# lh3/minigraph

Measured on NVIDIA H100. Metric: mapped Gbp/s (-cx lr), higher is better.
Workload: dtype int64/u8 (fp32 chain penalties, bit-exact)

## Files before the change

### minigraph_b200/csrc/mgb_galign.cuh

```cuda
#pragma once
#include "mgb_pipeline.cuh"
#include "mgb_gchain.cuh"
#include "mgb_wfa_tiers.cuh"
#if defined(MGB_HOSTSIM)
#include <stdio.h>
#include <stdlib.h>
#endif

namespace mgb {

MG_HD inline int cigar_append1(Arena &A, AVec<uint64_t> &c, int32_t op, int32_t len)
{
	if (c.n > 0 && (int32_t)(c.a[c.n - 1] & 0xf) == op) c.a[c.n - 1] += (uint64_t)(int64_t)len << 4;
	else {
		uint64_t x = (uint64_t)(int64_t)len << 4 | (uint64_t)op;
		MGB_TRY(avec_push(A, c, x));
	}
	return 0;
}

MG_HD inline int cigar_append(Arena &A, AVec<uint64_t> &c, int32_t n_cigar, const uint32_t *cigar)
{
	if (n_cigar == 0) return 0;
	MGB_TRY(cigar_append1(A, c, (int32_t)(cigar[0] & 0xf), (int32_t)(cigar[0] >> 4)));
	MGB_TRY(avec_reserve(A, c, c.n + n_cigar - 1));
	for (int32_t k = 0; k < n_cigar - 1; ++k) c.a[c.n + k] = cigar[1 + k];
	c.n += n_cigar - 1;
	return 0;
}

struct CigarOut { uint64_t *cigar; int32_t n; };

struct WfaJob {
	int32_t rid, gc;
	int32_t l0, l;
	int32_t t_beg;
	int32_t t_last;
	int32_t tl, ql, q_off;
	int32_t n_cigar, status;
	int64_t lc_off;
	int64_t cig_off;
};

static const uint64_t PLAN_JOB = 1ULL << 63;
MG_HD inline unsigned long long *wfa_cig_chunk(int32_t *smem, int tier)
{
	static_assert(WfTier1::BYTES % 8 == 0 && WfTier1::BYTES + 16 <= WfTier1::STRIDE && WfTier2::BYTES % 8 == 0 && WfTier2::BYTES + 16 <= WfTier2::STRIDE, "no room for the slice state behind the tier layouts");
	return smem == 0 || tier > 2? (unsigned long long*)0 : (unsigned long long*)((char*)smem + (tier == 1? WfTier1::BYTES : WfTier2::BYTES));
}
static const unsigned long long CIG_CHUNK_BYTES = 2048;


MG_HD inline int wfa_job_run(Arena &A, const PipeCtx &c, int64_t job_idx, int lane, int32_t *smem, int tier, WfTbJob *tb)
{
	WfaJob *J = &c.jobs[job_idx];
	if (J->rid < 0) return 0;
	const int32_t rid = J->rid, l0 = J->l0, l = J->l, tl = J->tl, ql = J->ql;
	if (c.meta[rid].status < 0) return 0;
	const int32_t mlen = tl > ql? tl : ql;
	const int explore = (job_idx & 63) == 0;
	if (!explore && tier == 1 && mlen >= c.skip1_len) {
		if (lane == 0) {
			unsigned int at;
#if MGB_ON_DEVICE
			at = atomicAdd(&c.jobq_n[tier - 1], 1u);
#else
			at = c.jobq_n[tier - 1]++;
#endif
			c.jobq[tier - 1][at] = (int32_t)job_idx;
		}
		return 0;
	}
	const bool t2_long = tl > WfTier2::MAXLEN_ || ql > WfTier2::MAXLEN_;
	if ((tier == 1 && (tl > WfTier1::MAXLEN_ || ql > WfTier1::MAXLEN_)) || (tier == 2 && t2_long && !wf_ring_always_fits(tl, ql))) {
		if (lane == 0) {
			unsigned int at;
#if MGB_ON_DEVICE
			at = atomicAdd(&c.jobq_n[tier - 1], 1u);
#else
			at = c.jobq_n[tier - 1]++;
#endif
			c.jobq[tier - 1][at] = (int32_t)job_idx;
		}
		return 0;
	}
	const GraphDev &g = c.g;
	const LLChain *lc = (const LLChain*)(c.out + J->lc_off);
	const char *qs = c.b.seq + c.b.seq_off[rid] + J->q_off;
	const char *tseq;
	if (l == l0) tseq = g_vseq(g, lc[l0].v) + J->t_beg;
	else {
		char *seq;
		MGB_ALLOC(A, seq, char, tl + 1);
		int32_t n = g_vlen(g, lc[l0].v) - J->t_beg, at = 0;
		const char *s = g_vseq(g, lc[l0].v) + J->t_beg;
		for (int32_t x = lane; x < n; x += MGB_W) seq[at + x] = s[x];
		at += n;
		for (int32_t k = l0 + 1; k < l; ++k) {
			s = g_vseq(g, lc[k].v), n = g_vlen(g, lc[k].v);
			for (int32_t x = lane; x < n; x += MGB_W) seq[at + x] = s[x];
			at += n;
		}
		s = g_vseq(g, lc[l].v), n = J->t_last + 1;
		for (int32_t x = lane; x < n; x += MGB_W) seq[at + x] = s[x];
		at += n;
		if (at != tl) return MGB_E_INTERNAL;
		warp_sync();
		tseq = seq;
	}
	WfResult rst;
	unsigned long long pt0 = prof_clock();
	int rc;
	int64_t cont_cells = 0;
	if (tier == 1) rc = wfa_smem<WfTier1::W_, WfTier1::MAXLEN_, WfTier1::TBCAP_>(A, smem, tl, tseq, ql, qs, &rst, lane);
// ... 28 lines not shown
			c.jobq[tier - 1][at] = (int32_t)job_idx;
		}
		return 0;
	}
	if (rst.s < 0) return MGB_E_INTERNAL;
	wfa_tb_keep(tb, rst, tl, tseq, ql, qs, job_idx, lane);
	return 1;
}

MG_HD inline int wfa_job_finish(const PipeCtx &c, const WfTbJob &b, int32_t *smem, int tier, int lane)
{
	if (b.rc < 0) return b.rc;
	const int32_t n_cigar = b.n_cigar;
	const uint32_t *cigar = b.cig + b.first;
	int64_t coff = 0;
	if (lane == 0) {
#if MGB_ON_DEVICE
		unsigned long long *ck = wfa_cig_chunk(smem, tier);
		const unsigned long long need = ((unsigned long long)n_cigar * 4 + 15) & ~15ULL;
		if (ck == 0) coff = pool_alloc(c.pool_cig, (uint64_t)n_cigar * 4);
		else if (ck[0] + need > ck[1]) {
			const unsigned long long get = need > CIG_CHUNK_BYTES? need : CIG_CHUNK_BYTES;
			const int64_t off = pool_alloc(c.pool_cig, get);
			if (off < 0) ck[0] = ck[1] = 0;
			else ck[0] = (unsigned long long)off, ck[1] = (unsigned long long)off + get;
			coff = off;
		}
		if (ck && coff >= 0) coff = (int64_t)ck[0], ck[0] += need;
#else
		coff = pool_alloc(c.pool_cig, (uint64_t)n_cigar * 4);
#endif
	}
	coff = (int64_t)warp_bcast_u64((uint64_t)coff, 0);
	if (coff < 0) return MGB_E_POOL;
	uint32_t *dst = (uint32_t*)((char*)c.cig + coff);
	for (int32_t x = lane; x < n_cigar; x += MGB_W) dst[x] = cigar[x];
	if (lane == 0) { WfaJob *J = &c.jobs[b.job]; J->n_cigar = n_cigar, J->cig_off = coff; }
	return 0;
}

template<typename G>
struct WfaBatch {
	WfTbJob *rec;
	int32_t n;
	MG_HD void open(Arena &A)
	{
		A.top = 0, n = 0;
		rec = (WfTbJob*)arena_alloc(A, (uint64_t)MGB_W * sizeof(WfTbJob));
	}
	MG_HD void flush(const G &g, Arena &A, int lane)
	{
		if (n > 0) {
			const unsigned long long t0 = prof_clock();
			wfa_tb_batch(rec, n, lane);
			g.traced(prof_clock() - t0, lane);
			for (int32_t j = 0; j < n; ++j) {
				const WfTbJob &b = rec[j];
				const int rc = g.done(b, lane);
				if (rc < 0) g.fail(b.item, rc, lane);
			}
			warp_sync();
		}
		open(A);
	}
	MG_HD void add(const G &g, int item, Arena &A, int lane)
	{
		uint64_t mark = A.top;
		int rc = g.run(item, A, rec + n, lane);
		if (rc == MGB_E_ARENA && n > 0) {
			flush(g, A, lane);
			mark = A.top;
			rc = g.run(item, A, rec + n, lane);
		}
		if (rc < 0) g.fail(item, rc, lane);
		if (rc == 1) {
			if (lane == 0) rec[n].item = item;
			++n;
		} else A.top = mark;
		if (n == MGB_W || A.top > A.cap / 4) flush(g, A, lane);
	}
};


#if MGB_ON_DEVICE
MG_D inline void lane_atomic_add_u64(uint64_t *p, uint64_t v) { atomicAdd((unsigned long long*)p, (unsigned long long)v); }
#else
inline void lane_atomic_add_u64(uint64_t *p, uint64_t v) { *p += v; }
#endif

MG_HD inline int gchain_cigar_finish_w(Arena &A, const PipeCtx &c, GcSet &gt, CigarOut *out, int lane)
{
	const uint64_t FIRST = 1ULL << 62;
	for (int32_t i = 0; i < gt.n_gc; ++i) {
		GChain *gc = &gt.gc[i];
		const int32_t off_a0 = gt.lc[gc->off].off, n_plan = gc->n_plan;
		const uint64_t *plan = c.plan + gc->plan_off;
		int32_t *ioff;
		MGB_ALLOC(A, ioff, int32_t, n_plan + 1);
		int32_t tot = 0;
		for (int32_t base = 0; base < n_plan; base += MGB_W) {
			const int32_t t = base + lane;
			int32_t cnt = 0;
			if (t < n_plan) cnt = (plan[t] & PLAN_JOB)? c.jobs[plan[t] & ~PLAN_JOB].n_cigar : 1;
			const int32_t incl = warp_incl_scan_i32(cnt, lane);
			if (t < n_plan) ioff[t] = tot + incl - cnt;
			tot += warp_bcast_i32(incl, MGB_W - 1);
		}
		uint64_t *F, *O;
		int32_t *oidx;
		MGB_ALLOC(A, F, uint64_t, tot + 1);
		MGB_ALLOC(A, O, uint64_t, tot + 1);
		MGB_ALLOC(A, oidx, int32_t, tot + 1);
		warp_sync();
		for (int32_t t = lane; t < n_plan; t += MGB_W) {
			uint64_t *dst = F + ioff[t];
			if (plan[t] & PLAN_JOB) {
				const WfaJob *J = &c.jobs[plan[t] & ~PLAN_JOB];
				const uint32_t *cig = (const uint32_t*)((const char*)c.cig + J->cig_off);
				for (int32_t k = 0; k < J->n_cigar; ++k) dst[k] = (uint64_t)cig[k] | (k == 0? FIRST : 0);
			} else dst[0] = plan[t] | FIRST;
		}
		warp_sync();
		int32_t n_out = 0;
		for (int32_t base = 0; base < tot; base += MGB_W) {
			const int32_t j = base + lane;
			int head = 0;
			if (j < tot) head = j == 0 || !((F[j] & FIRST) && (F[j] & 0xf) == (F[j - 1] & 0xf));
			const uint32_t mh = warp_ballot(head);
			if (j < tot) {
				const int32_t o = n_out + mask_rank(mh, lane) + head - 1;
				oidx[j] = o;
				if (head) O[o] = F[j] & 0xf;
			}
			n_out += mask_count(mh);
		}
		warp_sync();
		for (int32_t j = lane; j < tot; j += MGB_W) lane_atomic_add_u64(&O[oidx[j]], (F[j] & ~FIRST) >> 4 << 4);
		warp_sync();
		int32_t mlen = 0, blen = 0, aplen = 0, l = 0;
		for (int32_t j = lane; j < n_out; j += MGB_W) {
			const int32_t op = (int32_t)(O[j] & 0xf), len = (int32_t)(O[j] >> 4);
			if (op == 7) mlen += len;
			blen += len;
			if (op != 1) aplen += len;
			if (op != 2) l += len;
		}
		mlen = warp_sum_i32(mlen), blen = warp_sum_i32(blen), aplen = warp_sum_i32(aplen), l = warp_sum_i32(l);
		if (lane == 0) {
			out[i].cigar = O, out[i].n = n_out;
			gc->has_cigar = 1;
			gc->n_cigar = n_out;
			gc->c_ss = (int32_t)gt.a[off_a0].x + 1 - (int32_t)(gt.a[off_a0].y >> 32 & 0xff);
			gc->c_ee = (int32_t)gt.a[off_a0 + gc->n_anchor - 1].x + 1;
			gc->c_mlen = mlen, gc->c_blen = blen, gc->c_aplen = aplen;
		}
		if (!(l == gc->qe - gc->qs && aplen == gc->pe - gc->ps)) return MGB_E_INTERNAL;
		warp_sync();
	}
	return 0;
}


struct DsOut { char *ds; int32_t len; int32_t *off; int32_t n_off; };

MG_HD inline char ds_nt(const char *s, int64_t i) { return "acgtn"[nt4((uint8_t)s[i])]; }

MG_HD inline char *ds_w_int(char *w, int32_t c)
{
	char buf[16];
	int l = 0;
	uint32_t x = c >= 0? (uint32_t)c : (uint32_t)(-c);
	do { buf[l++] = (char)(x % 10 + '0'); x /= 10; } while (x > 0);
	if (c < 0) buf[l++] = '-';
	for (int i = l - 1; i >= 0; --i) *w++ = buf[i];
	return w;
}

MG_HD inline char *ds_w_indel(char *w, int64_t len, const char *seq, int64_t ll, int64_t lr)
{
	int64_t i;
	if (ll + lr >= len) {
		*w++ = '[';
		for (i = 0; i < len; ++i) *w++ = ds_nt(seq, i);
		*w++ = ']';
	} else {
		int64_t k = 0;
		if (ll > 0) {
			*w++ = '[';
			for (i = 0; i < ll; ++i) *w++ = ds_nt(seq, k + i);
			*w++ = ']';
			k += ll;
		}
		for (i = 0; i < len - lr - ll; ++i) *w++ = ds_nt(seq, k + i);
		k += len - lr - ll;
		if (lr > 0) {
			*w++ = '[';
			for (i = 0; i < lr; ++i) *w++ = ds_nt(seq, k + i);
			*w++ = ']';
		}
	}
	return w;
}

static const int DS_CHUNKS = 32;
struct DsChunk { int64_t dx, dy; int32_t cap_b, cap_o, n_b, n_o; };

MG_HD inline int gchain_ds_w(Arena &A, const GraphDev &g, const char *qseq, GcSet &gt, const CigarOut *cg, DsOut *out, int lane)
{
	for (int32_t i = 0; i < gt.n_gc; ++i) {
		GChain *gc = &gt.gc[i];
		const uint64_t *cigar = cg[i].cigar;
		const int32_t n_cigar = gc->n_cigar, aplen = gc->c_aplen;
		char *seq;
		int64_t seq_l = 0;
		MGB_ALLOC(A, seq, char, aplen + 1);
		for (int32_t j = 0; j < gc->cnt; ++j) {
			const int32_t k = gc->off + j;
			const uint32_t v = gt.lc[k].v;
			const int32_t slen = g_vlen(g, v);
			const int32_t st = j > 0? 0 : gc->c_ss;
			const int32_t en = j < gc->cnt - 1? slen : gc->c_ee;
			if (seq_l + (en - st) > aplen) return MGB_E_INTERNAL;
			const char *s = g_vseq(g, v) + st;
			for (int32_t t = lane; t < en - st; t += MGB_W) seq[seq_l + t] = s[t];
			seq_l += en - st;
		}
		if (seq_l != aplen) return MGB_E_INTERNAL;
		DsChunk *ch;
		MGB_ALLOC(A, ch, DsChunk, DS_CHUNKS);
		const int32_t per = (n_cigar + DS_CHUNKS - 1) / DS_CHUNKS;
		for (int c = lane; c < DS_CHUNKS; c += MGB_W) {
			const int32_t j0 = c * per < n_cigar? c * per : n_cigar, j1 = j0 + per < n_cigar? j0 + per : n_cigar;
			DsChunk d;
			d.dx = d.dy = 0, d.cap_b = d.cap_o = d.n_b = d.n_o = 0;
			for (int32_t j = j0; j < j1; ++j) {
				const int64_t op = (int64_t)(cigar[j] & 0xf), len = (int64_t)(cigar[j] >> 4);
				if (op == 7) d.dx += len, d.dy += len, d.cap_b += 12, d.cap_o += 1;
				else if (op == 0 || op == 8) d.dx += len, d.dy += len, d.cap_b += (int32_t)(14 * len + 12), d.cap_o += (int32_t)(2 * len + 1);
				else if (op == 1) d.dy += len, d.cap_b += (int32_t)(len + 6), d.cap_o += 1;
				else if (op == 2) d.dx += len, d.cap_b += (int32_t)(len + 6), d.cap_o += 1;
			}
			ch[c] = d;
		}
		warp_sync();
		int64_t tot_cb = 0, tot_co = 0;
		for (int c = 0; c < DS_CHUNKS; ++c) tot_cb += ch[c].cap_b, tot_co += ch[c].cap_o;
		char *tmp_b;
		int32_t *tmp_o;
		MGB_ALLOC(A, tmp_b, char, tot_cb);
		MGB_ALLOC(A, tmp_o, int32_t, tot_co);
		int bad = 0;
		for (int c = lane; c < DS_CHUNKS; c += MGB_W) {
			const int32_t j0 = c * per < n_cigar? c * per : n_cigar, j1 = j0 + per < n_cigar? j0 + per : n_cigar;
			int64_t x = 0, y = gc->qs, cb = 0, co = 0;
			for (int q = 0; q < c; ++q) x += ch[q].dx, y += ch[q].dy, cb += ch[q].cap_b, co += ch[q].cap_o;
			char *const w0 = tmp_b + cb;
			char *w = w0;
			int32_t *const o0 = tmp_o + co;
			int32_t *o = o0;
			for (int32_t j = j0; j < j1; ++j) {
				const int64_t op = (int64_t)(cigar[j] & 0xf), len = (int64_t)(cigar[j] >> 4);
				if (op == 0 || op == 7 || op == 8) {
					int64_t z;
					int32_t l = 0;
					if (op == 7) l = (int32_t)len, z = len;
					else z = 0;
					for (; z < len; ++z) {
						const uint8_t cx = (uint8_t)nt4((uint8_t)seq[x + z]);
						const uint8_t cy = (uint8_t)nt4((uint8_t)qseq[y + z]);
						if (cx != cy) {
							if (l > 0) { *o++ = (int32_t)(w - w0); *w++ = ':'; w = ds_w_int(w, l); }
							*o++ = (int32_t)(w - w0);
							*w++ = '*', *w++ = "acgtn"[cx], *w++ = "acgtn"[cy];
							l = 0;
						} else ++l;
					}
					if (l > 0) { *o++ = (int32_t)(w - w0); *w++ = ':'; w = ds_w_int(w, l); }
					x += len, y += len;
				} else if (op == 1) {
					int64_t z, ll, lr;
					for (z = 1; z <= len; ++z)
						if (y - z < gc->qs || qseq[y + len - z] != qseq[y - z]) break;
					lr = z - 1;
					for (z = 0; z < len; ++z)
						if (y + len + z >= gc->qe || qseq[y + len + z] != qseq[y + z]) break;
					ll = z;
					*o++ = (int32_t)(w - w0);
					*w++ = '+';
					w = ds_w_indel(w, len, &qseq[y], ll, lr);
					y += len;
				} else if (op == 2) {
					int64_t z, ll, lr;
					for (z = 1; z <= len; ++z)
						if (x - z < 0 || seq[x + len - z] != seq[x - z]) break;
					lr = z - 1;
					for (z = 0; z < len; ++z)
						if (x + len + z >= aplen || seq[x + z] != seq[x + len + z]) break;
					ll = z;
					*o++ = (int32_t)(w - w0);
					*w++ = '-';
					w = ds_w_indel(w, len, &seq[x], ll, lr);
					x += len;
				}
			}
			ch[c].n_b = (int32_t)(w - w0), ch[c].n_o = (int32_t)(o - o0);
			if (ch[c].n_b > ch[c].cap_b || ch[c].n_o > ch[c].cap_o) bad = 1;
		}
		if (warp_any(bad)) return MGB_E_INTERNAL;
		warp_sync();
		int64_t tot_b = 0, tot_o = 0;
		for (int c = 0; c < DS_CHUNKS; ++c) tot_b += ch[c].n_b, tot_o += ch[c].n_o;
		char *str;
		int32_t *off;
		MGB_ALLOC(A, str, char, tot_b + 1);
		MGB_ALLOC(A, off, int32_t, tot_o);
		{
			int64_t cb = 0, co = 0, ab = 0, ao = 0;
			for (int c = 0; c < DS_CHUNKS; ++c) {
				const char *sb = tmp_b + cb;
				const int32_t *so = tmp_o + co;
				for (int32_t t = lane; t < ch[c].n_b; t += MGB_W) str[ab + t] = sb[t];
				for (int32_t t = lane; t < ch[c].n_o; t += MGB_W) off[ao + t] = so[t] + (int32_t)ab;
				cb += ch[c].cap_b, co += ch[c].cap_o, ab += ch[c].n_b, ao += ch[c].n_o;
			}
		}
		warp_sync();
		out[i].ds = str, out[i].len = (int32_t)tot_b, out[i].off = off, out[i].n_off = (int32_t)tot_o;
		if (lane == 0) gc->ds_len = (int32_t)tot_b, gc->n_dsoff = (int32_t)tot_o;
	}
	return 0;
}

struct ReadOut {
	int32_t status;
	int32_t n_gc, n_lc, n_a, rep_len;
	int32_t n_mz;
	uint32_t blob_size, blob2_size;
	int64_t blob_off;
	int64_t blob2_off;
};

MG_HD inline uint64_t align8(uint64_t x) { return (x + 7) & ~(uint64_t)7; }

struct GState {
	int32_t n_lc, n_u, n_gc, n_jobs;
	int64_t job_first;
};

MG_HD inline int stage_gchain_plan(const PipeCtx &c, ReadMeta &m, int rid, Arena &A, int32_t n_lc, LChain *lc, int32_t n_u, const uint64_t *u, const u128 *a, uint32_t *gc_hash)
{
	const MapOptDev &o = c.opt;
	int32_t n_gc = 0;
	int64_t job_first;
	{
		int64_t off = pool_alloc(c.pool_gjobs, (uint64_t)(n_lc > 0? n_lc : 1) * sizeof(GwfaJob));
		if (off < 0) return MGB_E_POOL;
		job_first = off / (int64_t)sizeof(GwfaJob);
	}
	struct LocalEmit {
		GwfaJob *dst; int rid; int32_t n, cap;
		MG_HD int operator()(GwfaJob &J) { if (n >= cap) return MGB_E_INTERNAL; J.rid = rid; dst[n++] = J; return 0; }
	} le;
	le.dst = c.gjobs + job_first, le.rid = rid, le.n = 0, le.cap = n_lc > 0? n_lc : 1;
	MGB_TRY(gchain_prep(c.g, n_u, u, lc, a, m.hash, o.min_gc_cnt, o.min_gc_score, o.gdp_max_ed, batch_n_seg(c.b, rid), gc_hash, &n_gc, le));
	for (int32_t i = le.n; i < le.cap; ++i) le.dst[i].rid = -1;
	uint64_t sz = sizeof(GState) + align8((uint64_t)n_lc * sizeof(LChain)) + (uint64_t)n_u * 8 + align8((uint64_t)n_gc * 4);
	int64_t goff = pool_alloc(c.pool_gstate, sz);
	if (goff < 0) return MGB_E_POOL;
	GState *gsb = (GState*)(c.gstate + goff);
	gsb->n_lc = n_lc, gsb->n_u = n_u, gsb->n_gc = n_gc, gsb->n_jobs = le.n, gsb->job_first = job_first;
	LChain *dlc = (LChain*)(gsb + 1);
	for (int32_t i = 0; i < n_lc; ++i) dlc[i] = lc[i];
	uint64_t *du = (uint64_t*)((char*)dlc + align8((uint64_t)n_lc * sizeof(LChain)));
	for (int32_t i = 0; i < n_u; ++i) du[i] = u[i];
	uint32_t *dh = (uint32_t*)(du + n_u);
	for (int32_t i = 0; i < n_gc; ++i) dh[i] = gc_hash[i];
	m.gstate_off = goff;
	return 0;
}

MG_HD inline int stage_gchain(const PipeCtx &c, ReadOut *routs, int rid, Arena &A, int lane)
{
	ReadMeta &m = c.meta[rid];
	ReadOut &ro = routs[rid];
	const MapOptDev &o = c.opt;
	if (lane == 0) ro.status = 0, ro.n_gc = ro.n_lc = ro.n_a = 0, ro.rep_len = m.rep_len, ro.n_mz = m.n_mz, ro.blob_size = ro.blob2_size = 0, ro.blob_off = ro.blob2_off = 0;
	if (m.status != 0) { if (lane == 0) ro.status = m.status; return 0; }
	const uint64_t mark = A.top;
	const int32_t qlen = c.b.seq_len[rid];
	const u128 *a = c.anchor + m.a_off;
	int32_t n_lc = m.n_lc, n_u = 0;
	uint64_t *u = 0;
	LChain *lc;
	uint32_t *gc_hash;
	MGB_ALLOC(A, lc, LChain, n_lc);
	MGB_ALLOC(A, gc_hash, uint32_t, n_lc);
	for (int32_t i = lane; i < n_lc; i += MGB_W) lc[i] = c.lchain[m.lc_off + i];
	warp_sync();
	unsigned long long pt0 = prof_clock();
	GcParam gp;
	gp.max_dist_g = gp.max_dist_q = gp.bw = o.bw_long, gp.ref_bonus = o.ref_bonus, gp.chn_pen_gap = o.chn_pen_gap, gp.mask_level = o.mask_level;
	MGB_TRY(gchain_dp_w(A, c.g, c.lab, &n_lc, lc, qlen, gp, o.max_gc_skip, a, &u, &n_u, lane));
	if (lane == 0) { unsigned long long dt = prof_clock() - pt0; prof_add(c, PROF_GC_DP_CYC, dt); prof_max(c, PROF_GC_DP_MAX_CYC, dt); }
	int rc = 0;
	if (lane == 0) {
		Arena B = A;
		rc = stage_gchain_plan(c, m, rid, B, n_lc, lc, n_u, u, a, gc_hash);
		if (B.peak > A.peak) A.peak = B.peak;
	}
	rc = warp_bcast_i32(rc, 0);
	A.top = mark;
	return rc;
}
// ... 136 lines not shown
	const MapOptDev &o = c.opt;
	if (m.status != 0) { ro.status = m.status; return 0; }
	uint64_t mark = A.top;
	const char *qseq = c.b.seq + c.b.seq_off[rid];
	const int32_t qlen = c.b.seq_len[rid];
	const u128 *a = c.anchor + m.a_off;
	const GState *gsb = (const GState*)(c.gstate + m.gstate_off);
	const int32_t n_lc = gsb->n_lc, n_u = gsb->n_u;
	LChain *lc;
	MGB_ALLOC(A, lc, LChain, n_lc);
	{
		const LChain *slc = (const LChain*)(gsb + 1);
		for (int32_t i = 0; i < n_lc; ++i) lc[i] = slc[i];
	}
	const uint64_t *u = (const uint64_t*)((const char*)(gsb + 1) + align8((uint64_t)n_lc * sizeof(LChain)));
	const uint32_t *gc_hash = (const uint32_t*)(u + n_u);
	GwfaFeed feed;
	feed.job = c.gjobs + gsb->job_first, feed.walk_pool = c.walk, feed.next = 0, feed.n = gsb->n_jobs;
	GcSet gs;
	unsigned long long pt1 = prof_clock();
	MGB_TRY(gchain_gen(A, c.g, n_u, u, lc, a, m.hash, o.min_gc_cnt, o.min_gc_score, o.gdp_max_ed, batch_n_seg(c.b, rid), qseq, gs, &feed, gc_hash));
	gs.rep_len = m.rep_len;
	unsigned long long pt2 = prof_clock();
	prof_add(c, PROF_GC_GEN_CYC, pt2 - pt1);
	prof_add(c, PROF_GC_SHORTK_CYC, gs.cyc_shortk), prof_add(c, PROF_GC_EXTRA_CYC, gs.cyc_extra);
	MGB_TRY(gchain_set_parent(A, o.mask_level, gs.n_gc, gs.gc, o.sub_diff));
	gchain_flt_sub(o.pri_ratio, c.ix.k * 2, o.best_n, gs.n_gc, gs.gc);
	MGB_TRY(gchain_drop_flt(A, gs));
	MGB_TRY(gchain_set_mapq(o, gs, qlen, m.n_mz, o.min_gc_score));
	unsigned long long pt3 = prof_clock();
	prof_add(c, PROF_GC_POST_CYC, pt3 - pt2);
	uint64_t off_lc = align8((uint64_t)gs.n_gc * sizeof(GChain));
	uint64_t off_a = off_lc + align8((uint64_t)gs.n_lc * sizeof(LLChain));
	uint64_t sz = off_a + align8((uint64_t)gs.n_a * sizeof(u128));
	int64_t boff = pool_alloc(c.pool_out, sz);
	if (boff < 0) return MGB_E_POOL;
	for (int32_t i = 0; i < gs.n_gc; ++i) {
		GChain *gc = &gs.gc[i];
		gc->has_cigar = 0, gc->n_cigar = 0, gc->cigar_off = gc->ds_off = gc->dsoff_off = 0, gc->ds_len = gc->n_dsoff = 0, gc->plan_off = 0, gc->n_plan = 0;
	}
	hand->gs = gs, hand->boff = boff, hand->off_lc = off_lc, hand->off_a = off_a, hand->sz = sz, hand->mark = mark, hand->pt3 = pt3;
	hand->want_plan = (o.flag & F_CIGAR) && gs.n_gc > 0 && batch_n_seg(c.b, rid) == 1, hand->skip = 0;
	return 0;
}

MG_HD inline int stage_gchain_gen(const PipeCtx &c, ReadOut *routs, int rid, Arena &A, int lane)
{
	GenHand h;
	h.gs.n_gc = h.gs.n_lc = h.gs.n_a = h.gs.rep_len = 0, h.gs.gc = 0, h.gs.lc = 0, h.gs.a = 0;
	h.gs.cyc_gwfa = h.gs.cyc_shortk = h.gs.cyc_extra = 0;
	h.boff = 0, h.off_lc = h.off_a = h.sz = 0, h.mark = A.top, h.pt3 = 0, h.want_plan = 0, h.skip = 1;
	int rc = 0;
	Arena B = A;
	if (lane == 0) rc = stage_gchain_gen_head(c, routs, rid, B, &h);
	rc = warp_bcast_i32(rc, 0);
	A.top = warp_bcast_u64(B.top, 0), A.peak = warp_bcast_u64(B.peak, 0);
	h.skip = warp_bcast_i32(h.skip, 0);
	warp_sync();
	if (rc < 0 || h.skip) { A.top = h.mark; return rc; }
	h.gs.n_gc = warp_bcast_i32(h.gs.n_gc, 0), h.gs.n_lc = warp_bcast_i32(h.gs.n_lc, 0), h.gs.n_a = warp_bcast_i32(h.gs.n_a, 0);
	h.gs.gc = (GChain*)warp_bcast_u64((uint64_t)h.gs.gc, 0), h.gs.lc = (LLChain*)warp_bcast_u64((uint64_t)h.gs.lc, 0), h.gs.a = (u128*)warp_bcast_u64((uint64_t)h.gs.a, 0);
	h.boff = (int64_t)warp_bcast_u64((uint64_t)h.boff, 0), h.off_lc = warp_bcast_u64(h.off_lc, 0), h.off_a = warp_bcast_u64(h.off_a, 0), h.sz = warp_bcast_u64(h.sz, 0);
	h.want_plan = warp_bcast_i32(h.want_plan, 0);
	if (h.want_plan) MGB_TRY(gchain_cigar_plan_w(A, c, rid, c.g, h.gs, h.boff + (int64_t)h.off_lc, lane));
	char *blob = c.out + h.boff;
	{
		GChain *d = (GChain*)blob;
		for (int32_t i = lane; i < h.gs.n_gc; i += MGB_W) d[i] = h.gs.gc[i];
		LLChain *dl = (LLChain*)(blob + h.off_lc);
		for (int32_t i = lane; i < h.gs.n_lc; i += MGB_W) dl[i] = h.gs.lc[i];
		u128 *da = (u128*)(blob + h.off_a);
		for (int32_t i = lane; i < h.gs.n_a; i += MGB_W) da[i] = h.gs.a[i];
	}
	if (lane == 0) {
		ReadOut &ro = routs[rid];
		ro.n_gc = h.gs.n_gc, ro.n_lc = h.gs.n_lc, ro.n_a = h.gs.n_a, ro.blob_size = (uint32_t)h.sz, ro.blob_off = h.boff;
		prof_add(c, PROF_GC_PLAN_CYC, prof_clock() - h.pt3);
	}
	warp_sync();
	A.top = h.mark;
	return 0;
}

MG_HD inline int stage_finish(const PipeCtx &c, ReadOut *routs, int rid, Arena &A, int lane)
{
	ReadMeta &m = c.meta[rid];
	ReadOut &ro = routs[rid];
	if (m.status != 0) { if (lane == 0) ro.status = m.status; return 0; }
	if (!(c.opt.flag & F_CIGAR) || ro.n_gc == 0 || batch_n_seg(c.b, rid) != 1) return 0;
	uint64_t mark = A.top;
	const char *qseq = c.b.seq + c.b.seq_off[rid];
	char *blob = c.out + ro.blob_off;
	GcSet gs;
	gs.n_gc = ro.n_gc, gs.n_lc = ro.n_lc, gs.n_a = ro.n_a, gs.rep_len = ro.rep_len;
	gs.gc = (GChain*)blob;
	gs.lc = (LLChain*)(blob + align8((uint64_t)gs.n_gc * sizeof(GChain)));
	gs.a = (u128*)((char*)gs.lc + align8((uint64_t)gs.n_lc * sizeof(LLChain)));
	CigarOut *cg;
	DsOut *ds;
	MGB_ALLOC(A, cg, CigarOut, gs.n_gc);
	MGB_ALLOC(A, ds, DsOut, gs.n_gc);
	unsigned long long pt0 = prof_clock();
	MGB_TRY(gchain_cigar_finish_w(A, c, gs, cg, lane));
	unsigned long long pt1 = prof_clock();
	MGB_TRY(gchain_ds_w(A, c.g, qseq, gs, cg, ds, lane));
	if (lane == 0) prof_add(c, PROF_FIN_CIGAR_CYC, pt1 - pt0), prof_add(c, PROF_FIN_DS_CYC, prof_clock() - pt1);
	uint64_t sz = 0;
	for (int32_t i = 0; i < gs.n_gc; ++i)
		sz += align8((uint64_t)cg[i].n * 8) + align8((uint64_t)ds[i].len + 1) + align8((uint64_t)ds[i].n_off * 4);
	int64_t boff = 0;
	if (lane == 0) boff = pool_alloc(c.pool_out, sz);
	boff = (int64_t)warp_bcast_u64((uint64_t)boff, 0);
	if (boff < 0) return MGB_E_POOL;
	uint64_t at = (uint64_t)boff;
	for (int32_t i = 0; i < gs.n_gc; ++i) {
		GChain *gc = &gs.gc[i];
		const int64_t cigar_off = (int64_t)at; at += align8((uint64_t)cg[i].n * 8);
		const int64_t ds_off = (int64_t)at; at += align8((uint64_t)ds[i].len + 1);
		const int64_t dsoff_off = (int64_t)at; at += align8((uint64_t)ds[i].n_off * 4);
		if (lane == 0) gc->cigar_off = cigar_off, gc->ds_off = ds_off, gc->dsoff_off = dsoff_off;
		uint64_t *dc = (uint64_t*)(c.out + cigar_off);
		for (int32_t k = lane; k < cg[i].n; k += MGB_W) dc[k] = cg[i].cigar[k];
		char *dd = c.out + ds_off;
		for (int32_t k = lane; k < ds[i].len; k += MGB_W) dd[k] = ds[i].ds[k];
		if (lane == 0) dd[ds[i].len] = 0;
		int32_t *dof = (int32_t*)(c.out + dsoff_off);
		for (int32_t k = lane; k < ds[i].n_off; k += MGB_W) dof[k] = ds[i].off[k];
	}
	if (lane == 0) ro.blob2_off = boff, ro.blob2_size = (uint32_t)sz;
	A.top = mark;
	return 0;
}

}
```

Before: 1.478.

## Rewrite finish stage: fused per-lane cigar merge and two-pass per-op ds generation

The cigar merge no longer builds a flattened array with atomics. Each lane binary-searches the plan offsets to find its op, and runs are merged with warp scans, writing the merged ops directly. The ds string is now built with one op per lane in two passes, a counting pass and a writing pass that goes straight into the output pool, replacing the 32-chunk staging buffers and final copies. Long indels get warp-cooperative flank search and writing. This removes staging copies and serial per-chunk work. In exchange the op lookup becomes more complex, and lanes diverge when op lengths vary.

```diff
diff --git a/minigraph_b200/csrc/mgb_galign.cuh b/minigraph_b200/csrc/mgb_galign.cuh
--- a/minigraph_b200/csrc/mgb_galign.cuh
+++ b/minigraph_b200/csrc/mgb_galign.cuh
@@ -28,8 +28,6 @@
 	c.n += n_cigar - 1;
 	return 0;
 }
-
-struct CigarOut { uint64_t *cigar; int32_t n; };
 
 struct WfaJob {
 	int32_t rid, gc;
@@ -224,253 +222,215 @@
 };
 
 
+MG_HD inline int mask_lowest(uint32_t m)
+{
 #if MGB_ON_DEVICE
-MG_D inline void lane_atomic_add_u64(uint64_t *p, uint64_t v) { atomicAdd((unsigned long long*)p, (unsigned long long)v); }
+	return __ffs(m) - 1;
 #else
-inline void lane_atomic_add_u64(uint64_t *p, uint64_t v) { *p += v; }
+	return __builtin_ctz(m);
 #endif
-
-MG_HD inline int gchain_cigar_finish_w(Arena &A, const PipeCtx &c, GcSet &gt, CigarOut *out, int lane)
-{
-	const uint64_t FIRST = 1ULL << 62;
-	for (int32_t i = 0; i < gt.n_gc; ++i) {
-		GChain *gc = &gt.gc[i];
-		const int32_t off_a0 = gt.lc[gc->off].off, n_plan = gc->n_plan;
-		const uint64_t *plan = c.plan + gc->plan_off;
-		int32_t *ioff;
-		MGB_ALLOC(A, ioff, int32_t, n_plan + 1);
-		int32_t tot = 0;
-		for (int32_t base = 0; base < n_plan; base += MGB_W) {
-			const int32_t t = base + lane;
-			int32_t cnt = 0;
-			if (t < n_plan) cnt = (plan[t] & PLAN_JOB)? c.jobs[plan[t] & ~PLAN_JOB].n_cigar : 1;
-			const int32_t incl = warp_incl_scan_i32(cnt, lane);
-			if (t < n_plan) ioff[t] = tot + incl - cnt;
-			tot += warp_bcast_i32(incl, MGB_W - 1);
-		}
-		uint64_t *F, *O;
-		int32_t *oidx;
-		MGB_ALLOC(A, F, uint64_t, tot + 1);
-		MGB_ALLOC(A, O, uint64_t, tot + 1);
-		MGB_ALLOC(A, oidx, int32_t, tot + 1);
-		warp_sync();
-		for (int32_t t = lane; t < n_plan; t += MGB_W) {
-			uint64_t *dst = F + ioff[t];
-			if (plan[t] & PLAN_JOB) {
-				const WfaJob *J = &c.jobs[plan[t] & ~PLAN_JOB];
-				const uint32_t *cig = (const uint32_t*)((const char*)c.cig + J->cig_off);
-				for (int32_t k = 0; k < J->n_cigar; ++k) dst[k] = (uint64_t)cig[k] | (k == 0? FIRST : 0);
-			} else dst[0] = plan[t] | FIRST;
-		}
-		warp_sync();
-		int32_t n_out = 0;
-		for (int32_t base = 0; base < tot; base += MGB_W) {
-			const int32_t j = base + lane;
-			int head = 0;
-			if (j < tot) head = j == 0 || !((F[j] & FIRST) && (F[j] & 0xf) == (F[j - 1] & 0xf));
-			const uint32_t mh = warp_ballot(head);
-			if (j < tot) {
-				const int32_t o = n_out + mask_rank(mh, lane) + head - 1;
-				oidx[j] = o;
-				if (head) O[o] = F[j] & 0xf;
+}
+
+MG_HD inline int gchain_cigar_finish_w(Arena &A, const PipeCtx &c, GcSet &gt, int32_t i, uint64_t **ops, int lane)
+{
+	GChain *gc = &gt.gc[i];
+	const int32_t off_a0 = gt.lc[gc->off].off, n_plan = gc->n_plan;
+	const uint64_t *plan = c.plan + gc->plan_off;
+	int32_t *ioff;
+	MGB_ALLOC(A, ioff, int32_t, n_plan + 1);
+	int32_t tot = 0;
+	for (int32_t base = 0; base < n_plan; base += MGB_W) {
+		const int32_t t = base + lane;
+		int32_t cnt = 0;
+		if (t < n_plan) cnt = (plan[t] & PLAN_JOB)? c.jobs[plan[t] & ~PLAN_JOB].n_cigar : 1;
+		const int32_t incl = warp_incl_scan_i32(cnt, lane);
+		if (t < n_plan) ioff[t] = tot + incl - cnt;
+		tot += warp_bcast_i32(incl, MGB_W - 1);
+	}
+	uint64_t *O;
+	MGB_ALLOC(A, O, uint64_t, tot);
+	warp_sync();
+	int32_t n_out = 0, t_lo = 0, carry = 0, prev_op = 0, mlen = 0, blen = 0, aplen = 0, l = 0;
+	for (int32_t base = 0; base < tot; base += MGB_W) {
+		const int32_t j = base + lane;
+		int32_t t = t_lo, op = 0, len = 0, first = 0;
+		if (j < tot) {
+			for (int32_t hi = n_plan - 1; t < hi; ) {
+				const int32_t mid = (t + hi + 1) >> 1;
+				if (ioff[mid] <= j) t = mid;
+				else hi = mid - 1;
 			}
-			n_out += mask_count(mh);
-		}
-		warp_sync();
-		for (int32_t j = lane; j < tot; j += MGB_W) lane_atomic_add_u64(&O[oidx[j]], (F[j] & ~FIRST) >> 4 << 4);
-		warp_sync();
-		int32_t mlen = 0, blen = 0, aplen = 0, l = 0;
-		for (int32_t j = lane; j < n_out; j += MGB_W) {
-			const int32_t op = (int32_t)(O[j] & 0xf), len = (int32_t)(O[j] >> 4);
+			uint64_t v = plan[t];
+			if (v & PLAN_JOB) {
+				const WfaJob *J = &c.jobs[v & ~PLAN_JOB];
+				v = ((const uint32_t*)((const char*)c.cig + J->cig_off))[j - ioff[t]];
+			}
+			op = (int32_t)(v & 0xf), len = (int32_t)(v >> 4), first = j == ioff[t];
 			if (op == 7) mlen += len;
 			blen += len;
 			if (op != 1) aplen += len;
 			if (op != 2) l += len;
 		}
-		mlen = warp_sum_i32(mlen), blen = warp_sum_i32(blen), aplen = warp_sum_i32(aplen), l = warp_sum_i32(l);
-		if (lane == 0) {
-			out[i].cigar = O, out[i].n = n_out;
-			gc->has_cigar = 1;
-			gc->n_cigar = n_out;
-			gc->c_ss = (int32_t)gt.a[off_a0].x + 1 - (int32_t)(gt.a[off_a0].y >> 32 & 0xff);
-			gc->c_ee = (int32_t)gt.a[off_a0 + gc->n_anchor - 1].x + 1;
-			gc->c_mlen = mlen, gc->c_blen = blen, gc->c_aplen = aplen;
-		}
-		if (!(l == gc->qe - gc->qs && aplen == gc->pe - gc->ps)) return MGB_E_INTERNAL;
-		warp_sync();
-	}
+		const int32_t up = (int32_t)warp_shfl_up1_u64((uint64_t)(uint32_t)op);
+		const int32_t left = lane > 0? up : prev_op;
+		const int head = j < tot && (j == 0 || !(first && op == left));
+		const uint32_t mh = warp_ballot(head);
+		const int32_t incl = warp_incl_scan_i32(len, lane);
+		const uint64_t hs = warp_incl_scan_max_u64(head? (uint64_t)(incl - len) + 1 : 0, lane);
+		const int32_t run = hs? incl - (int32_t)(hs - 1) : carry + incl;
+		const int32_t o = n_out + mask_rank(mh, lane) + head - 1;
+		if (j < tot && (lane == MGB_W - 1 || j == tot - 1 || (mh >> (lane + 1) & 1))) O[o] = (uint64_t)(int64_t)run << 4 | (uint64_t)op;
+		carry = warp_bcast_i32(run, MGB_W - 1), prev_op = warp_bcast_i32(op, MGB_W - 1), t_lo = warp_bcast_i32(t, MGB_W - 1);
+		n_out += mask_count(mh);
+	}
+	mlen = warp_sum_i32(mlen), blen = warp_sum_i32(blen), aplen = warp_sum_i32(aplen), l = warp_sum_i32(l);
+	if (lane == 0) {
+		gc->has_cigar = 1;
+		gc->n_cigar = n_out;
+		gc->c_ss = (int32_t)gt.a[off_a0].x + 1 - (int32_t)(gt.a[off_a0].y >> 32 & 0xff);
+		gc->c_ee = (int32_t)gt.a[off_a0 + gc->n_anchor - 1].x + 1;
+		gc->c_mlen = mlen, gc->c_blen = blen, gc->c_aplen = aplen;
+	}
+	if (!(l == gc->qe - gc->qs && aplen == gc->pe - gc->ps)) return MGB_E_INTERNAL;
+	warp_sync();
+	*ops = O;
 	return 0;
 }
 
 
-struct DsOut { char *ds; int32_t len; int32_t *off; int32_t n_off; };
-
 MG_HD inline char ds_nt(const char *s, int64_t i) { return "acgtn"[nt4((uint8_t)s[i])]; }
-
-MG_HD inline char *ds_w_int(char *w, int32_t c)
-{
-	char buf[16];
-	int l = 0;
-	uint32_t x = c >= 0? (uint32_t)c : (uint32_t)(-c);
-	do { buf[l++] = (char)(x % 10 + '0'); x /= 10; } while (x > 0);
-	if (c < 0) buf[l++] = '-';
-	for (int i = l - 1; i >= 0; --i) *w++ = buf[i];
-	return w;
-}
-
-MG_HD inline char *ds_w_indel(char *w, int64_t len, const char *seq, int64_t ll, int64_t lr)
-{
-	int64_t i;
-	if (ll + lr >= len) {
-		*w++ = '[';
-		for (i = 0; i < len; ++i) *w++ = ds_nt(seq, i);
-		*w++ = ']';
-	} else {
-		int64_t k = 0;
-		if (ll > 0) {
-			*w++ = '[';
-			for (i = 0; i < ll; ++i) *w++ = ds_nt(seq, k + i);
-			*w++ = ']';
-			k += ll;
-		}
-		for (i = 0; i < len - lr - ll; ++i) *w++ = ds_nt(seq, k + i);
-		k += len - lr - ll;
-		if (lr > 0) {
-			*w++ = '[';
-			for (i = 0; i < lr; ++i) *w++ = ds_nt(seq, k + i);
-			*w++ = ']';
-		}
-	}
-	return w;
-}
-
-static const int DS_CHUNKS = 32;
-struct DsChunk { int64_t dx, dy; int32_t cap_b, cap_o, n_b, n_o; };
-
-MG_HD inline int gchain_ds_w(Arena &A, const GraphDev &g, const char *qseq, GcSet &gt, const CigarOut *cg, DsOut *out, int lane)
-{
-	for (int32_t i = 0; i < gt.n_gc; ++i) {
-		GChain *gc = &gt.gc[i];
-		const uint64_t *cigar = cg[i].cigar;
-		const int32_t n_cigar = gc->n_cigar, aplen = gc->c_aplen;
-		char *seq;
-		int64_t seq_l = 0;
-		MGB_ALLOC(A, seq, char, aplen + 1);
-		for (int32_t j = 0; j < gc->cnt; ++j) {
-			const int32_t k = gc->off + j;
-			const uint32_t v = gt.lc[k].v;
-			const int32_t slen = g_vlen(g, v);
-			const int32_t st = j > 0? 0 : gc->c_ss;
-			const int32_t en = j < gc->cnt - 1? slen : gc->c_ee;
-			if (seq_l + (en - st) > aplen) return MGB_E_INTERNAL;
-			const char *s = g_vseq(g, v) + st;
-			for (int32_t t = lane; t < en - st; t += MGB_W) seq[seq_l + t] = s[t];
-			seq_l += en - st;
-		}
-		if (seq_l != aplen) return MGB_E_INTERNAL;
-		DsChunk *ch;
-		MGB_ALLOC(A, ch, DsChunk, DS_CHUNKS);
-		const int32_t per = (n_cigar + DS_CHUNKS - 1) / DS_CHUNKS;
-		for (int c = lane; c < DS_CHUNKS; c += MGB_W) {
-			const int32_t j0 = c * per < n_cigar? c * per : n_cigar, j1 = j0 + per < n_cigar? j0 + per : n_cigar;
-			DsChunk d;
-			d.dx = d.dy = 0, d.cap_b = d.cap_o = d.n_b = d.n_o = 0;
-			for (int32_t j = j0; j < j1; ++j) {
-				const int64_t op = (int64_t)(cigar[j] & 0xf), len = (int64_t)(cigar[j] >> 4);
-				if (op == 7) d.dx += len, d.dy += len, d.cap_b += 12, d.cap_o += 1;
-				else if (op == 0 || op == 8) d.dx += len, d.dy += len, d.cap_b += (int32_t)(14 * len + 12), d.cap_o += (int32_t)(2 * len + 1);
-				else if (op == 1) d.dy += len, d.cap_b += (int32_t)(len + 6), d.cap_o += 1;
-				else if (op == 2) d.dx += len, d.cap_b += (int32_t)(len + 6), d.cap_o += 1;
+MG_HD inline int32_t ds_ndig(uint32_t x) { int32_t n = 1; while (x >= 10) x /= 10, ++n; return n; }
+MG_HD inline void ds_put_int(char *w, uint32_t x, int32_t n) { for (int32_t k = n - 1; k >= 0; --k) w[k] = (char)('0' + x % 10), x /= 10; }
+
+MG_HD inline int32_t ds_match(char *w, int32_t *off, int32_t b0, int32_t op, int32_t len, const char *t, const char *q, int32_t *n_off)
+{
+	int32_t nb = 0, no = 0, l = 0, z = 0;
+	if (op == 7) l = len, z = len;
+	for (; z < len; ++z) {
+		const int cx = nt4((uint8_t)t[z]), cy = nt4((uint8_t)q[z]);
+		if (cx != cy) {
+			if (l > 0) {
+				const int32_t d = ds_ndig((uint32_t)l);
+				if (w) off[no] = b0 + nb, w[nb] = ':', ds_put_int(w + nb + 1, (uint32_t)l, d);
+				++no, nb += 1 + d;
 			}
-			ch[c] = d;
-		}
-		warp_sync();
-		int64_t tot_cb = 0, tot_co = 0;
-		for (int c = 0; c < DS_CHUNKS; ++c) tot_cb += ch[c].cap_b, tot_co += ch[c].cap_o;
-		char *tmp_b;
-		int32_t *tmp_o;
-		MGB_ALLOC(A, tmp_b, char, tot_cb);
-		MGB_ALLOC(A, tmp_o, int32_t, tot_co);
-		int bad = 0;
-		for (int c = lane; c < DS_CHUNKS; c += MGB_W) {
-			const int32_t j0 = c * per < n_cigar? c * per : n_cigar, j1 = j0 + per < n_cigar? j0 + per : n_cigar;
-			int64_t x = 0, y = gc->qs, cb = 0, co = 0;
-			for (int q = 0; q < c; ++q) x += ch[q].dx, y += ch[q].dy, cb += ch[q].cap_b, co += ch[q].cap_o;
-			char *const w0 = tmp_b + cb;
-			char *w = w0;
-			int32_t *const o0 = tmp_o + co;
-			int32_t *o = o0;
-			for (int32_t j = j0; j < j1; ++j) {
-				const int64_t op = (int64_t)(cigar[j] & 0xf), len = (int64_t)(cigar[j] >> 4);
-				if (op == 0 || op == 7 || op == 8) {
-					int64_t z;
-					int32_t l = 0;
-					if (op == 7) l = (int32_t)len, z = len;
-					else z = 0;
-					for (; z < len; ++z) {
-						const uint8_t cx = (uint8_t)nt4((uint8_t)seq[x + z]);
-						const uint8_t cy = (uint8_t)nt4((uint8_t)qseq[y + z]);
-						if (cx != cy) {
-							if (l > 0) { *o++ = (int32_t)(w - w0); *w++ = ':'; w = ds_w_int(w, l); }
-							*o++ = (int32_t)(w - w0);
-							*w++ = '*', *w++ = "acgtn"[cx], *w++ = "acgtn"[cy];
-							l = 0;
-						} else ++l;
-					}
-					if (l > 0) { *o++ = (int32_t)(w - w0); *w++ = ':'; w = ds_w_int(w, l); }
-					x += len, y += len;
-				} else if (op == 1) {
-					int64_t z, ll, lr;
-					for (z = 1; z <= len; ++z)
-						if (y - z < gc->qs || qseq[y + len - z] != qseq[y - z]) break;
-					lr = z - 1;
-					for (z = 0; z < len; ++z)
-						if (y + len + z >= gc->qe || qseq[y + len + z] != qseq[y + z]) break;
-					ll = z;
-					*o++ = (int32_t)(w - w0);
-					*w++ = '+';
-					w = ds_w_indel(w, len, &qseq[y], ll, lr);
-					y += len;
-				} else if (op == 2) {
-					int64_t z, ll, lr;
-					for (z = 1; z <= len; ++z)
-						if (x - z < 0 || seq[x + len - z] != seq[x - z]) break;
-					lr = z - 1;
-					for (z = 0; z < len; ++z)
-						if (x + len + z >= aplen || seq[x + z] != seq[x + len + z]) break;
-					ll = z;
-					*o++ = (int32_t)(w - w0);
-					*w++ = '-';
-					w = ds_w_indel(w, len, &seq[x], ll, lr);
-					x += len;
-				}
-			}
-			ch[c].n_b = (int32_t)(w - w0), ch[c].n_o = (int32_t)(o - o0);
-			if (ch[c].n_b > ch[c].cap_b || ch[c].n_o > ch[c].cap_o) bad = 1;
-		}
-		if (warp_any(bad)) return MGB_E_INTERNAL;
-		warp_sync();
-		int64_t tot_b = 0, tot_o = 0;
-		for (int c = 0; c < DS_CHUNKS; ++c) tot_b += ch[c].n_b, tot_o += ch[c].n_o;
-		char *str;
-		int32_t *off;
-		MGB_ALLOC(A, str, char, tot_b + 1);
-		MGB_ALLOC(A, off, int32_t, tot_o);
-		{
-			int64_t cb = 0, co = 0, ab = 0, ao = 0;
-			for (int c = 0; c < DS_CHUNKS; ++c) {
-				const char *sb = tmp_b + cb;
-				const int32_t *so = tmp_o + co;
-				for (int32_t t = lane; t < ch[c].n_b; t += MGB_W) str[ab + t] = sb[t];
-				for (int32_t t = lane; t < ch[c].n_o; t += MGB_W) off[ao + t] = so[t] + (int32_t)ab;
-				cb += ch[c].cap_b, co += ch[c].cap_o, ab += ch[c].n_b, ao += ch[c].n_o;
-			}
-		}
-		warp_sync();
-		out[i].ds = str, out[i].len = (int32_t)tot_b, out[i].off = off, out[i].n_off = (int32_t)tot_o;
-		if (lane == 0) gc->ds_len = (int32_t)tot_b, gc->n_dsoff = (int32_t)tot_o;
-	}
-	return 0;
+			if (w) off[no] = b0 + nb, w[nb] = '*', w[nb + 1] = "acgtn"[cx], w[nb + 2] = "acgtn"[cy];
+			++no, nb += 3, l = 0;
+		} else ++l;
+	}
+	if (l > 0) {
+		const int32_t d = ds_ndig((uint32_t)l);
+		if (w) off[no] = b0 + nb, w[nb] = ':', ds_put_int(w + nb + 1, (uint32_t)l, d);
+		++no, nb += 1 + d;
+	}
+	*n_off = no;
+	return nb;
+}
+
+MG_HD inline void ds_flanks(const char *s, int32_t p, int32_t len, int32_t lo, int32_t hi, int32_t *ll, int32_t *lr)
+{
+	int32_t z;
+	for (z = 1; z <= len; ++z)
+		if (p - z < lo || s[p + len - z] != s[p - z]) break;
+	*lr = z - 1;
+	for (z = 0; z < len; ++z)
+		if (p + len + z >= hi || s[p + len + z] != s[p + z]) break;
+	*ll = z;
+}
+MG_HD inline void ds_flanks_w(const char *s, int32_t p, int32_t len, int32_t lo, int32_t hi, int32_t *ll, int32_t *lr, int lane)
+{
+	*lr = *ll = len;
+	for (int32_t z0 = 1; z0 <= len; z0 += MGB_W) {
+		const int32_t z = z0 + lane;
+		const uint32_t m = warp_ballot(z <= len && (p - z < lo || s[p + len - z] != s[p - z]));
+		if (m) { *lr = z0 + mask_lowest(m) - 1; break; }
+	}
+	for (int32_t z0 = 0; z0 < len; z0 += MGB_W) {
+		const int32_t z = z0 + lane;
+		const uint32_t m = warp_ballot(z < len && (p + len + z >= hi || s[p + len + z] != s[p + z]));
+		if (m) { *ll = z0 + mask_lowest(m); break; }
+	}
+}
+
+MG_HD inline int32_t ds_indel_bytes(int32_t len, int32_t ll, int32_t lr) { return 1 + (ll + lr >= len? len + 2 : len + (ll > 0? 2 : 0) + (lr > 0? 2 : 0)); }
+MG_HD inline char ds_indel_char(int32_t r, int32_t op, int32_t len, const char *s, int32_t ll, int32_t lr)
+{
+	if (r == 0) return op == 1? '+' : '-';
+	r -= 1;
+	if (ll + lr >= len) return r == 0? '[' : r == len + 1? ']' : ds_nt(s, r - 1);
+	const int32_t a = ll > 0? ll + 2 : 0;
+	if (r < a) return r == 0? '[' : r == a - 1? ']' : ds_nt(s, r - 1);
+	r -= a;
+	if (r < len - ll - lr) return ds_nt(s, ll + r);
+	r -= len - ll - lr;
+	return r == 0? '[' : r == lr + 1? ']' : ds_nt(s, len - lr + r - 1);
+}
+
+static const int32_t DS_LONG_INDEL = 32;
+
+template<bool WRITE>
+MG_HD inline void gchain_ds_pass_w(const uint64_t *ops, int32_t n_cigar, uint64_t *at, const char *seq, int32_t aplen, const char *qseq, int32_t qs, int32_t qe,
+                                   uint64_t *dc, char *ds, int32_t *dof, int32_t *ds_len, int32_t *n_off, int lane)
+{
+	int32_t x0 = 0, y0 = qs, b_tot = 0, o_tot = 0;
+	for (int32_t base = 0; base < n_cigar; base += MGB_W) {
+		const int32_t j = base + lane;
+		int32_t op = -1, len = 0;
+		if (j < n_cigar) {
+			const uint64_t v = ops[j];
+			op = (int32_t)(v & 0xf), len = (int32_t)(v >> 4);
+			if (WRITE) dc[j] = v;
+		}
+		const int match = op == 0 || op == 7 || op == 8, indel = op == 1 || op == 2;
+		const int32_t dx = match || op == 2? len : 0, dy = match || op == 1? len : 0;
+		const int32_t ix = warp_incl_scan_i32(dx, lane), iy = warp_incl_scan_i32(dy, lane);
+		const int32_t x = x0 + ix - dx, y = y0 + iy - dy;
+		x0 += warp_bcast_i32(ix, MGB_W - 1), y0 += warp_bcast_i32(iy, MGB_W - 1);
+		const char *s = op == 1? qseq : seq;
+		const int32_t p = op == 1? y : x, lo = op == 1? qs : 0, hi = op == 1? qe : aplen;
+		const int is_long = indel && len >= DS_LONG_INDEL;
+		const uint32_t m_long = warp_ballot(is_long);
+		int32_t ll = 0, lr = 0;
+		for (uint32_t m = m_long; m; m &= m - 1) {
+			const int src = mask_lowest(m);
+			const int32_t sop = warp_bcast_i32(op, src), slen = warp_bcast_i32(len, src), sp = warp_bcast_i32(p, src);
+			int32_t a, b;
+			ds_flanks_w(sop == 1? qseq : seq, sp, slen, sop == 1? qs : 0, sop == 1? qe : aplen, &a, &b, lane);
+			if (lane == src) ll = a, lr = b;
+		}
+		if (indel && !is_long) ds_flanks(s, p, len, lo, hi, &ll, &lr);
+		int32_t b0, o0;
+		if (!WRITE) {
+			int32_t nb = 0, no = 0;
+			if (indel) nb = ds_indel_bytes(len, ll, lr), no = 1;
+			else if (match) nb = ds_match(0, 0, 0, op, len, seq + x, qseq + y, &no);
+			const int32_t ib = warp_incl_scan_i32(nb, lane), io = warp_incl_scan_i32(no, lane);
+			b0 = b_tot + ib - nb, o0 = o_tot + io - no;
+			if (j < n_cigar) at[j] = (uint64_t)(uint32_t)o0 << 32 | (uint32_t)b0;
+			b_tot += warp_bcast_i32(ib, MGB_W - 1), o_tot += warp_bcast_i32(io, MGB_W - 1);
+			continue;
+		}
+		b0 = o0 = 0;
+		if (j < n_cigar) { const uint64_t v = at[j]; b0 = (int32_t)(uint32_t)v, o0 = (int32_t)(v >> 32); }
+		if (indel && !is_long) {
+			const int32_t nb = ds_indel_bytes(len, ll, lr);
+			dof[o0] = b0;
+			for (int32_t r = 0; r < nb; ++r) ds[b0 + r] = ds_indel_char(r, op, len, s + p, ll, lr);
+		} else if (match) {
+			int32_t no;
+			ds_match(ds + b0, dof + o0, b0, op, len, seq + x, qseq + y, &no);
+		}
+		for (uint32_t m = m_long; m; m &= m - 1) {
+			const int src = mask_lowest(m);
+			const int32_t sop = warp_bcast_i32(op, src), slen = warp_bcast_i32(len, src), sp = warp_bcast_i32(p, src), sb0 = warp_bcast_i32(b0, src);
+			const int32_t sll = warp_bcast_i32(ll, src), slr = warp_bcast_i32(lr, src);
+			const char *ss = (sop == 1? qseq : seq) + sp;
+			const int32_t nb = ds_indel_bytes(slen, sll, slr);
+			for (int32_t r = lane; r < nb; r += MGB_W) ds[sb0 + r] = ds_indel_char(r, sop, slen, ss, sll, slr);
+			if (lane == src) dof[o0] = b0;
+		}
+	}
+	*ds_len = b_tot, *n_off = o_tot;
 }
 
 struct ReadOut {
@@ -773,6 +733,8 @@
 	return 0;
 }
 
+struct FinChain { uint64_t *ops, *at; char *seq; };
+
 MG_HD inline int stage_finish(const PipeCtx &c, ReadOut *routs, int rid, Arena &A, int lane)
 {
 	ReadMeta &m = c.meta[rid];
@@ -780,6 +742,7 @@
 	if (m.status != 0) { if (lane == 0) ro.status = m.status; return 0; }
 	if (!(c.opt.flag & F_CIGAR) || ro.n_gc == 0 || batch_n_seg(c.b, rid) != 1) return 0;
 	uint64_t mark = A.top;
+	const GraphDev &g = c.g;
 	const char *qseq = c.b.seq + c.b.seq_off[rid];
 	char *blob = c.out + ro.blob_off;
 	GcSet gs;
@@ -787,37 +750,60 @@
 	gs.gc = (GChain*)blob;
 	gs.lc = (LLChain*)(blob + align8((uint64_t)gs.n_gc * sizeof(GChain)));
 	gs.a = (u128*)((char*)gs.lc + align8((uint64_t)gs.n_lc * sizeof(LLChain)));
-	CigarOut *cg;
-	DsOut *ds;
-	MGB_ALLOC(A, cg, CigarOut, gs.n_gc);
-	MGB_ALLOC(A, ds, DsOut, gs.n_gc);
+	FinChain *fc;
+	MGB_ALLOC(A, fc, FinChain, gs.n_gc);
 	unsigned long long pt0 = prof_clock();
-	MGB_TRY(gchain_cigar_finish_w(A, c, gs, cg, lane));
+	for (int32_t i = 0; i < gs.n_gc; ++i) {
+		uint64_t *ops;
+		MGB_TRY(gchain_cigar_finish_w(A, c, gs, i, &ops, lane));
+		if (lane == 0) fc[i].ops = ops;
+	}
 	unsigned long long pt1 = prof_clock();
-	MGB_TRY(gchain_ds_w(A, c.g, qseq, gs, cg, ds, lane));
-	if (lane == 0) prof_add(c, PROF_FIN_CIGAR_CYC, pt1 - pt0), prof_add(c, PROF_FIN_DS_CYC, prof_clock() - pt1);
 	uint64_t sz = 0;
-	for (int32_t i = 0; i < gs.n_gc; ++i)
-		sz += align8((uint64_t)cg[i].n * 8) + align8((uint64_t)ds[i].len + 1) + align8((uint64_t)ds[i].n_off * 4);
+	for (int32_t i = 0; i < gs.n_gc; ++i) {
+		GChain *gc = &gs.gc[i];
+		const int32_t aplen = gc->c_aplen, n_cigar = gc->n_cigar;
+		char *seq;
+		uint64_t *at;
+		MGB_ALLOC(A, seq, char, aplen + 1);
+		MGB_ALLOC(A, at, uint64_t, n_cigar);
+		int64_t seq_l = 0;
+		for (int32_t j = 0; j < gc->cnt; ++j) {
+			const uint32_t v = gs.lc[gc->off + j].v;
+			const int32_t st = j > 0? 0 : gc->c_ss;
+			const int32_t en = j < gc->cnt - 1? g_vlen(g, v) : gc->c_ee;
+			if (seq_l + (en - st) > aplen) return MGB_E_INTERNAL;
+			const char *s = g_vseq(g, v) + st;
+			for (int32_t t = lane; t < en - st; t += MGB_W) seq[seq_l + t] = s[t];
+			seq_l += en - st;
+		}
+		if (seq_l != aplen) return MGB_E_INTERNAL;
+		warp_sync();
+		int32_t ds_len, n_off;
+		gchain_ds_pass_w<false>(fc[i].ops, n_cigar, at, seq, aplen, qseq, gc->qs, gc->qe, 0, 0, 0, &ds_len, &n_off, lane);
+		sz += align8((uint64_t)n_cigar * 8) + align8((uint64_t)ds_len + 1) + align8((uint64_t)n_off * 4);
+		warp_sync();
+		if (lane == 0) fc[i].at = at, fc[i].seq = seq, gc->ds_len = ds_len, gc->n_dsoff = n_off;
+	}
 	int64_t boff = 0;
 	if (lane == 0) boff = pool_alloc(c.pool_out, sz);
 	boff = (int64_t)warp_bcast_u64((uint64_t)boff, 0);
 	if (boff < 0) return MGB_E_POOL;
+	warp_sync();
 	uint64_t at = (uint64_t)boff;
 	for (int32_t i = 0; i < gs.n_gc; ++i) {
 		GChain *gc = &gs.gc[i];
-		const int64_t cigar_off = (int64_t)at; at += align8((uint64_t)cg[i].n * 8);
-		const int64_t ds_off = (int64_t)at; at += align8((uint64_t)ds[i].len + 1);
-		const int64_t dsoff_off = (int64_t)at; at += align8((uint64_t)ds[i].n_off * 4);
-		if (lane == 0) gc->cigar_off = cigar_off, gc->ds_off = ds_off, gc->dsoff_off = dsoff_off;
-		uint64_t *dc = (uint64_t*)(c.out + cigar_off);
-		for (int32_t k = lane; k < cg[i].n; k += MGB_W) dc[k] = cg[i].cigar[k];
+		const int32_t n_cigar = gc->n_cigar, ds_len = gc->ds_len, n_off = gc->n_dsoff;
+		const int64_t cigar_off = (int64_t)at; at += align8((uint64_t)n_cigar * 8);
+		const int64_t ds_off = (int64_t)at; at += align8((uint64_t)ds_len + 1);
+		const int64_t dsoff_off = (int64_t)at; at += align8((uint64_t)n_off * 4);
 		char *dd = c.out + ds_off;
-		for (int32_t k = lane; k < ds[i].len; k += MGB_W) dd[k] = ds[i].ds[k];
-		if (lane == 0) dd[ds[i].len] = 0;
-		int32_t *dof = (int32_t*)(c.out + dsoff_off);
-		for (int32_t k = lane; k < ds[i].n_off; k += MGB_W) dof[k] = ds[i].off[k];
-	}
+		int32_t wl, wo;
+		gchain_ds_pass_w<true>(fc[i].ops, n_cigar, fc[i].at, fc[i].seq, gc->c_aplen, qseq, gc->qs, gc->qe, (uint64_t*)(c.out + cigar_off), dd, (int32_t*)(c.out + dsoff_off), &wl, &wo, lane);
+		warp_sync();
+		if (lane == 0) gc->cigar_off = cigar_off, gc->ds_off = ds_off, gc->dsoff_off = dsoff_off, dd[ds_len] = 0;
+	}
+	if (lane == 0) prof_add(c, PROF_FIN_CIGAR_CYC, pt1 - pt0), prof_add(c, PROF_FIN_DS_CYC, prof_clock() - pt1);
 	if (lane == 0) ro.blob2_off = boff, ro.blob2_size = (uint32_t)sz;
 	A.top = mark;
 	return 0;
```

Result: faster. 1.553, median of 6 (+5.1%).
